# samholt/NeuralLaplaceControl

Measured on AMD Instinct MI355X. Metric: MPPI planning steps/sec (16384 samples, H=40), higher is better.
Workload: dtype f64

## Files before the change

neurallaplacecontrol_amd/csrc/abi_ctx.hip:

```cpp
#include "nlc_host.h"

using namespace nlc;
using namespace nlc::host;

namespace nlc {
namespace host {

thread_local std::string g_create_error;

bool gru_use_coop(const nlc_ctx* c, int64_t n_windows) {
  if (c->opt.gru_coop >= 0) return c->opt.gru_coop != 0;
  if (c->g == 128) return true;
  return n_windows <= (c->g == 32 ? 8192 : 50000);
}

void prof_flush(nlc_ctx* c) {
  for (auto& p : c->prof) {
    for (auto& ev : p.pending) {
      hipEventSynchronize(ev.second);
      float ms = 0.f;
      hipEventElapsedTime(&ms, ev.first, ev.second);
      p.total_ms += ms;
      c->event_pool.push_back(ev.first);
      c->event_pool.push_back(ev.second);
// ... 178 lines not shown
  } else if (n == "fused_partner_tiles") {
    if (value < -2 || value > 64) return fail(c, NLC_ERR_BAD_ARG, "fused_partner_tiles must be in -2..64 (-2 = auto, -1 = never)");
    c->opt.fused.partner_tiles = (int)value;
  } else if (n == "repfunc_split") {
    if (value != 0 && value != 1) return fail(c, NLC_ERR_BAD_ARG, "repfunc_split must be 0 or 1");
    c->opt.repfunc_split = (int)value;
  } else if (n == "gru_coop") {
    if (value != 0 && value != 1 && value != -1) return fail(c, NLC_ERR_BAD_ARG, "gru_coop must be -1 (auto), 0 or 1");
    c->opt.gru_coop = (int)value;
  } else if (n == "gru_prefix") {
    if (value != 0 && value != 1 && value != -1) return fail(c, NLC_ERR_BAD_ARG, "gru_prefix must be -1 (auto), 0 or 1");
    c->opt.gru_prefix = (int)value;
  } else if (n == "gru_gemm") {
    if (value != 0 && value != 1) return fail(c, NLC_ERR_BAD_ARG, "gru_gemm must be 0 (FP64 MFMA) or 1 (int8-sliced)");
    c->opt.gru_gemm = (int)value;
    if (c->has_model) c->gru.use_i8 = (c->gru.i8_stream != nullptr && value == 1) ? 1 : 0;
  } else if (n == "dbg_gap_us") {
    if (value < 0 || value > 1.0e5) return fail(c, NLC_ERR_BAD_ARG, "dbg_gap_us must be in 0 .. 1e5");
    c->opt.dbg_gap_us = value;
  } else if (n == "dbg_l2_mb") {
    if (value < 0 || value > 4096) return fail(c, NLC_ERR_BAD_ARG, "dbg_l2_mb must be in 0 .. 4096");
    c->opt.dbg_l2_mb = value;
  } else if (n == "fused_max_samples") {
    if (value < 0) return fail(c, NLC_ERR_BAD_ARG, "fused_max_samples must be >= 0");
    c->opt.fused_max_samples = (int64_t)value;
  } else {
    return fail(c, NLC_ERR_BAD_ARG, "unknown option: " + n);
  }
  return NLC_OK;
}

extern "C" int nlc_get_stat(nlc_ctx* c, const char* name, double* out) {
  if (!c) return NLC_ERR_BAD_ARG;
  if (!name || !out) return fail(c, NLC_ERR_BAD_ARG, "NULL stat name / out");
  const std::string n(name);
  if (n == "rollout_body") *out = (double)c->last_body;
  else if (n == "fused_timeouts") *out = (double)c->fused.timeouts;
  else if (n == "fused_fallbacks") *out = (double)c->fused.fallbacks;
  else if (n == "fused_lost") *out = c->fused.lost ? 1.0 : 0.0;
  else if (n == "last_giveup_command") *out = (double)c->fused.last_giveup_command;
  else if (n == "commands") *out = (double)c->commands;
  else if (n == "comm_world") *out = c->comm ? (double)c->comm_world : 0.0;
  else if (n == "comm_rank") *out = c->comm ? (double)c->comm_rank : -1.0;
  else if (n == "fused_blocks_per_cu") *out = (double)c->fused.blocks_per_cu;
  else if (n == "fused_spin_limit") *out = (double)c->opt.fused_spin_limit;
  else if (n == "model_nt3") *out = c->has_model ? (double)c->net.nt3 : 0.0;
  else if (n == "gru_gemm") *out = (c->has_model && c->gru.use_i8) ? 1.0 : 0.0;
  else if (n == "gru_prefix") *out = c->prefix.last_used ? 1.0 : 0.0;
  else if (n.rfind("gru_prefix_windows_l", 0) == 0 && n.size() == 21 && n[20] >= '0' && n[20] <= '4') {
    *out = 0.0;
    if (c->prefix.last_used && c->prefix.lists) {
      unsigned cnt[nlc::prefix::kLists] = {0};
      NLC_HIP(c, hipStreamSynchronize(c->stream));
      NLC_HIP(c, hipMemcpy(cnt, c->prefix.lists, sizeof(cnt), hipMemcpyDeviceToHost));
      *out = (double)cnt[n[20] - '0'];
    }
  } else if (n == "gru_prefix_table_tiles") {
    *out = 0.0;
    if (c->prefix.last_used && c->prefix.lists) {
      unsigned cnt[nlc::prefix::kLists] = {0};
      NLC_HIP(c, hipStreamSynchronize(c->stream));
      NLC_HIP(c, hipMemcpy(cnt, c->prefix.lists, sizeof(cnt), hipMemcpyDeviceToHost));
      for (int l = 1; l < nlc::prefix::n_lists(c->prefix.last_B); ++l) *out += (double)((cnt[l] + 15u) / 16u);
    }
  } else if (n == "latents_offset") *out = (c->has_mppi && c->pd.dynamics == NLC_DYN_NL) ? (double)ws_layout(c).pa : -1.0;
  else if (n == "gru_i8_launches") *out = (double)nlc::gru_i8_launch_count();
  else return fail(c, NLC_ERR_BAD_ARG, "unknown stat: " + n);
  return NLC_OK;
}

extern "C" int nlc_synchronize(nlc_ctx* c) {
  if (!c) return NLC_ERR_BAD_ARG;
  NLC_HIP(c, hipStreamSynchronize(c->stream));
  return NLC_OK;
}

extern "C" int nlc_device_info(nlc_ctx* c, char* name, int name_len, int* cus, int* mhz, double* gib) {
  if (!c) return NLC_ERR_BAD_ARG;
  if (name && name_len > 0) {
    std::snprintf(name, name_len, "%s (%s)", c->prop.name, c->prop.gcnArchName);
  }
  if (cus) *cus = c->prop.multiProcessorCount;
  if (mhz) *mhz = c->prop.clockRate / 1000;
  if (gib) *gib = (double)c->prop.totalGlobalMem / (1024.0 * 1024.0 * 1024.0);
  return NLC_OK;
}

extern "C" int nlc_profile_enable(nlc_ctx* c, int on) {
  if (!c) return NLC_ERR_BAD_ARG;
  if (!on) prof_flush(c);
  c->profiling = on != 0;
  return NLC_OK;
}
extern "C" int nlc_profile_reset(nlc_ctx* c) {
  if (!c) return NLC_ERR_BAD_ARG;
  prof_flush(c);
  c->prof.clear();
  return NLC_OK;
}
extern "C" int nlc_profile_count(nlc_ctx* c) {
  if (!c) return NLC_ERR_BAD_ARG;
  return (int)c->prof.size();
}
extern "C" int nlc_profile_read(nlc_ctx* c, int idx, char* name, int name_len, double* total_ms, int64_t* launches) {
  if (!c) return NLC_ERR_BAD_ARG;
  if (idx < 0 || idx >= (int)c->prof.size()) return fail(c, NLC_ERR_BAD_ARG, "profile index out of range");
  prof_flush(c);
  const ProfEntry& p = c->prof[idx];
  if (name && name_len > 0) std::snprintf(name, name_len, "%s", p.name.c_str());
  if (total_ms) *total_ms = p.total_ms;
  if (launches) *launches = p.launches;
  return NLC_OK;
}
```

neurallaplacecontrol_amd/csrc/abi_planner.hip:

```cpp
#include "nlc_host.h"

using namespace nlc;
using namespace nlc::host;

extern "C" int nlc_mppi_configure(nlc_ctx* c, const nlc_mppi_desc* d) {
  if (!c) return NLC_ERR_BAD_ARG;
  NLC_GUARD_BEGIN
  if (!d) return fail(c, NLC_ERR_BAD_ARG, "NULL desc");
  if (d->K < 1 || d->T < 1 || d->K_global < d->K || d->k_offset < 0 || d->k_offset + d->K > d->K_global)
    return fail(c, NLC_ERR_BAD_SHAPE, "bad K / K_global / k_offset / T");
  if (d->nu < 1 || d->nu > NLC_MAX_NU) return fail(c, NLC_ERR_UNSUPPORTED, "nu must be 1 or 2");
  if (d->d < 1 || (d->d > NLC_MAX_D && d->dynamics != NLC_DYN_EXTERNAL)) return fail(c, NLC_ERR_BAD_SHAPE, "bad nx");
  if (d->B < 1) return fail(c, NLC_ERR_BAD_SHAPE, "action_buffer needs at least one row");
  if (!(d->lambda_ > 0.0) || d->u_scale == 0.0) return fail(c, NLC_ERR_BAD_ARG, "lambda_ must be > 0, u_scale != 0");
  if (d->u_per_command < 1 || d->u_per_command > d->T) return fail(c, NLC_ERR_BAD_ARG, "bad u_per_command");
  if (d->E < 0 || d->E > 65535) return fail(c, NLC_ERR_BAD_ARG, "episodes E must be in [0, 65535]");
  const int E = d->E < 1 ? 1 : d->E;
  if ((double)E * (double)d->K * d->T * d->nu > 2.0e9)
    return fail(c, NLC_ERR_BAD_SHAPE, "E*K*T*nu exceeds the planner's index range");
  const bool env_free = d->cost_external &&
                        (d->dynamics == NLC_DYN_NL || d->dynamics == NLC_DYN_DTRNN || d->dynamics == NLC_DYN_NODE) &&
                        d->env == -1;
  if (!env_free && (d->env < 0 || d->env > NLC_ENV_CARTPOLE_NOTRIG)) return fail(c, NLC_ERR_UNSUPPORTED, "unknown env id");
  static const int env_d[4] = {5, 3, 6, 4}, env_nu[4] = {1, 1, 2, 1};
// ... 142 lines not shown
  }
  if (g.lost_here || (g.marked && count_marked)) c->fused.last_giveup_command = command;
  return g;
}

WeightArgs make_weight_args(nlc_ctx* c, const nlc_mppi_buffers* buf) {
  const nlc_mppi_desc& d = c->pd;
  const WsLayout w = ws_layout(c);
  double* ws = (double*)buf->workspace;
  WeightArgs wa{};
  wa.Kep = d.K;
  wa.E = d.E;
  wa.T = d.T;
  wa.nu = d.nu;
  wa.lambda_ = d.lambda_;
  wa.cost = buf->cost_total;
  wa.noise = buf->noise;
  wa.tile_part = ws + w.tile_part;
  wa.chunk_part = ws + w.chunk_part;
  wa.partials = buf->partials;
  wa.nblk = c->nblk;
  return wa;
}

int finish_rollout_costs(nlc_ctx* c, const nlc_mppi_buffers* buf, bool in_body) {
  const nlc_mppi_desc& d = c->pd;
  if (d.cost_external) return NLC_OK;
  if (cost_variant_of(d) && !in_body) {
    if (!buf->states) return fail(c, NLC_ERR_BAD_ARG, "this rollout body evaluates a cost_variant on buf->states");
    VariantCostArgs v{d.K * d.E, d.T, d.nu, d.d, d.env, cost_variant_of(d), d.u_scale, buf->states, buf->perturbed, buf->cost_total};
    ProfScope ps(c, "variant_cost_kernel");
    NLC_HIP(c, launch_variant_cost(v, c->stream));
  }
  return run_weights(c, buf);
}

int run_weights(nlc_ctx* c, const nlc_mppi_buffers* buf) {
  WeightArgs wa = make_weight_args(c, buf);
  if (c->last_body == 3 && buf->workspace && c->pd.dynamics == NLC_DYN_NL)
    wa.gave_up = reinterpret_cast<const unsigned*>((const double*)buf->workspace + ws_layout(c).sync) + kFusedTimeout;
  ProfScope ps(c, "weight_kernels");
  NLC_HIP(c, launch_weights(wa, c->stream));
  return NLC_OK;
}

int launch_shift_perturb(nlc_ctx* c, RolloutCall& call) {
  PerturbArgs& p = call.p;
  p.fused_shift = (int64_t)p.K * p.T > 0;
  if (!p.fused_shift) {
    ProfScope ps(c, "shift_U_kernel");
    NLC_HIP(c, launch_shift_U(p, c->stream));
  }
  ProfScope ps(c, "perturb_kernel");
  NLC_HIP(c, launch_perturb(p, c->stream));
  return NLC_OK;
}

SampleCostArgs sample_cost_args(const nlc_ctx* c, const RolloutCall& call) {
  const nlc_mppi_desc& d = c->pd;
  SampleCostArgs a{};
  a.K = call.KE;
  a.Kep = d.K;
  a.T = d.T;
  a.nu = d.nu;
  a.env = (d.cost_external || cost_variant_of(d)) ? -1 : d.env;
  a.state_per_sample = call.state_per_sample;
  a.state0 = call.state_dev;
  a.perturbed = call.buf->perturbed;
  a.noise = call.buf->noise;
  a.U = c->U[c->ucur];
  for (int i = 0; i < NLC_MAX_NU * NLC_MAX_NU; ++i) a.sigma_inv[i] = d.noise_sigma_inv[i];
  a.lambda_ = d.lambda_;
  a.u_scale = d.u_scale;
  a.noise_abs_cost = d.noise_abs_cost;
  a.states = call.buf->states;
  a.cost_total = call.buf->cost_total;
  return a;
}

PerturbArgs perturb_args(const nlc_ctx* c, const nlc_mppi_buffers* buf, int rng, uint64_t seed, uint64_t counter) {
  const nlc_mppi_desc& d = c->pd;
  PerturbArgs p{};
  p.K = d.K * d.E;
  p.Kep = d.K;
  p.E = d.E;
  p.K_global = d.K_global;
  p.k_offset = d.k_offset;
  p.T = d.T;
  p.nu = d.nu;
  p.U_old = c->U[c->ucur];
  p.U_new = c->U[c->ucur ^ 1];
  p.noise = buf->noise;
  p.perturbed = buf->perturbed;
  p.actions = buf->actions;
  p.u_scale = d.u_scale;
  p.has_bounds = d.has_bounds;
  p.sample_null_action = d.sample_null_action;
  p.rng = rng;
  for (int i = 0; i < NLC_MAX_NU; ++i) {
    p.u_min[i] = d.u_min[i];
    p.u_max[i] = d.u_max[i];
    p.u_init[i] = d.u_init[i];
    p.mu[i] = d.noise_mu[i];
  }
  for (int i = 0; i < NLC_MAX_NU * NLC_MAX_NU; ++i) p.chol[i] = d.noise_chol[i];
  p.seed = seed;
  p.counter = counter;
// ... 370 lines not shown
```

neurallaplacecontrol_amd/csrc/abi_planner_nl.hip:

```cpp
#include "nlc_host.h"

using namespace nlc;
using namespace nlc::host;

namespace {

__global__ void dbg_spin_kernel(unsigned long long ticks_100mhz) {
  const unsigned long long t0 = __builtin_amdgcn_s_memrealtime();
  while (__builtin_amdgcn_s_memrealtime() - t0 < ticks_100mhz) __builtin_amdgcn_s_sleep(8);
}
__global__ void dbg_touch_kernel(const double* __restrict__ p, size_t n, double* __restrict__ sink) {
  double acc = 0.0;
  for (size_t i = (size_t)blockIdx.x * blockDim.x + threadIdx.x; i < n; i += (size_t)gridDim.x * blockDim.x) acc += p[i];
  if (acc == 12345.678) *sink = acc;
}
int dbg_between(nlc_ctx* c) {
  if (c->opt.dbg_gap_us > 0.0) hipLaunchKernelGGL(dbg_spin_kernel, dim3(1), dim3(64), 0, c->stream, (unsigned long long)(c->opt.dbg_gap_us * 100.0));
  if (c->opt.dbg_l2_mb > 0.0) {
    const size_t bytes = (size_t)(c->opt.dbg_l2_mb * 1048576.0);
    const size_t n = bytes / 8 + 1;
    if (c->dbg_scratch_n < n) {
      if (int rc = hold_doubles(c, c->dbg_scratch, n, nullptr, &c->dbg_scratch_n)) return rc;
      NLC_HIP(c, hipMemsetAsync(c->dbg_scratch, 0, n * sizeof(double), c->stream));
    }
// ... 291 lines not shown
  f.g.N = KE * d.T;
  FusedCtl& fc = f.ctl;
  fc.sync = reinterpret_cast<unsigned*>(ws + w.sync);
  fc.timeout_host = pin_giveup_word(c);
  fc.ntk = s.ntk;
  fc.n_enc = s.n_enc;
  fc.roll_cap = s.roll_cap;
  fc.adaptive_q8 = s.adaptive_q8;
  fc.pool_wgs = s.pool_wgs;
  fc.chain_first_tiles = s.chain_first_tiles;
  fc.partner_tiles = s.partner_tiles;
  fc.spin_limit = (unsigned)c->opt.fused_spin_limit;
  fc.test_drop_tile = c->opt.fused_test_drop_tile;
  fc.inline_weights = (c->opt.fused_inline & 1) && d.E == 1 && !d.cost_external;
  fc.inline_perturb = (c->opt.fused_inline & 2) && d.E == 1 && inline_inputs && rng == 1 && d.B <= kFusedMaxInlineB;
  unsigned* sync_words = reinterpret_cast<unsigned*>(ws + w.sync);
  const size_t n_sync = fused_sync_words(d.T, KE);
  if (fc.inline_perturb) {
    if (c->fused.sync_clean_ws != buf->workspace) NLC_HIP(c, hipMemsetAsync(sync_words, 0, n_sync * sizeof(unsigned), c->stream));
  } else {
    p.zero_words = sync_words;
    p.n_zero_words = (int64_t)n_sync;
    if (int rc = launch_shift_perturb(c, call)) return rc;
  }
  c->fused.sync_clean_ws = nullptr;
  c->fused.sync_dirty = true;
  c->fused.last.fused = true;
  c->last_body = 3;
  f.p = p;
  if (fc.inline_weights) f.w = make_weight_args(c, buf);
  {
    ProfScope ps(c, "nl_plan_fused_kernel");
    NLC_HIP(c, launch_nl_plan_fused(f, c->g, s.grid, s.built, c->stream));
  }
  *weights_done = fc.inline_weights != 0;
  return NLC_OK;
}

int gru_prefix_begin(nlc_ctx* c, RolloutCall& call, const GruArgs& g, int64_t N, int chunks, bool* use, GruPrefixArgs* px) {
  *use = false;
  if (c->opt.gru_prefix == 0) return NLC_OK;
  GruPrefixState& ps = c->prefix;
  const char* why = ps.why_not;
  if (!why && ps.last_B != g.B) why = "gru_prefix: the table was built for another action-buffer length";
  if (!why && chunks != 1) why = "gru_prefix: not with the encoder in horizon chunks (horizon_chunks)";
  if (!why && gru_use_coop(c, N)) why = "gru_prefix: this launch takes the cooperative encoder (gru_coop)";
  if (!why && g.use_i8) why = "gru_prefix: the FP64 encoder only (gru_gemm is 1)";
  if (!why) why = prefix::out_of_scope(g.nact, g.nin, 1, g.B, N, true);
  if (why) return c->opt.gru_prefix == 1 ? fail(c, NLC_ERR_UNSUPPORTED, why) : NLC_OK;
  const int64_t stride = (N + 63) / 64 * 64;
  const size_t need = 64 + (size_t)prefix::kLists * (size_t)stride / 2;
  if (need > ps.lists_n) {
    NLC_HIP(c, hipStreamSynchronize(c->stream));
    if (int rc = hold_doubles(c, ps.lists, need, nullptr, &ps.lists_n)) return rc;
  }
  double* base = c->arena.base + ps.arena_off;
  px->table = base;
  px->out_tab = base + (size_t)prefix::kEntries * 2 * c->g;
  px->products = base + gru_prefix_products_off(c->g);
  px->counts = reinterpret_cast<unsigned*>(ps.lists);
  px->lists = reinterpret_cast<unsigned*>(ps.lists + 64);
  px->list_stride = stride;
  px->img_max = ps.img_max;
  px->img_min = ps.img_min;
  call.p.zero_words = px->counts;
  call.p.n_zero_words = 16;
  *use = true;
  return NLC_OK;
}

int rollout_nl_two_launch(nlc_ctx* c, RolloutCall& call, GruArgs& g, RolloutArgs& r, int variant) {
  const nlc_mppi_desc& d = c->pd;
  const int64_t KE = call.KE;
  bool use_prefix = false;
  GruPrefixArgs px{};
  {
    const int chunks = plan::horizon_chunks((variant != 2 && KE > 8192 && d.E == 1) ? c->opt.horizon_chunks : 1, d.T).C;
    if (int rc = gru_prefix_begin(c, call, g, KE * d.T, chunks, &use_prefix, &px)) return rc;
  }
  if (int rc2 = nlc::host::launch_shift_perturb(c, call)) return rc2;
  const plan::Chunks ck = plan::horizon_chunks((variant != 2 && KE > 8192 && d.E == 1) ? c->opt.horizon_chunks : 1, d.T);
  const int C = ck.C, Tc = ck.Tc;
  if (C == 1) {
    g.t0 = 0;
    g.Tc = d.T;
    g.N = KE * d.T;
    if (use_prefix) {
      {
        ProfScope ps(c, "gru_prefix_index_kernel");
        NLC_HIP(c, launch_gru_prefix_index(g, px, c->stream));
      }
      ProfScope ps(c, "gru_encode_kernel");
      NLC_HIP(c, launch_gru_encode_prefix(g, px, c->g, c->stream));
      c->prefix.last_used = true;
    } else {
      ProfScope ps(c, "gru_encode_kernel");
      NLC_HIP(c, launch_gru_encode(g, c->g, c->stream, gru_use_coop(c, g.N)));
    }
    if (c->opt.dbg_gap_us > 0.0 || c->opt.dbg_l2_mb > 0.0)
      if (int rc3 = dbg_between(c)) return rc3;
    r.t_begin = 0;
    r.t_end = d.T;
    ProfScope ps(c, "nl_rollout_kernel");
    NLC_HIP(c, launch_nl_rollout(r, c->stream, variant));
  } else {
    if (int rc = gru_encode_chunks(c, g, KE, C, Tc, false, 0u)) return rc;
    for (int ch = 0; ch < C; ++ch) {
      r.t_begin = ch * Tc;
      r.t_end = (r.t_begin + Tc <= d.T) ? r.t_begin + Tc : d.T;
      if (r.t_begin >= r.t_end) break;
      NLC_HIP(c, hipStreamWaitEvent(c->stream, c->side.ev_gru[ch], 0));
      ProfScope ps(c, "nl_rollout_kernel");
      NLC_HIP(c, launch_nl_rollout(r, c->stream, 1));
    }
  }
  return NLC_OK;
}

}

int nlc::host::gru_prefix_configure(nlc_ctx* c) {
  const nlc_mppi_desc& d = c->pd;
  GruPrefixState& ps = c->prefix;
  ps.last_B = d.B;
  ps.last_used = false;
  const double img[2] = {prefix::bound_image(d.u_max[0], d.u_scale), prefix::bound_image(d.u_min[0], d.u_scale)};
  bool finite = true;
  for (double v : img) finite = finite && std::isfinite((d.u_scale * v - c->gru.mean[0]) / c->gru.std[0]);
  ps.why_not = prefix::out_of_scope(d.nu, c->md.nin, d.has_bounds, d.B, 0, finite);
  if (ps.why_not) return NLC_OK;
  ps.img_max = prefix::bits_of(img[0]);
  ps.img_min = prefix::bits_of(img[1]);
  std::vector<double> syn((size_t)16 * d.B, 0.0);
  for (int col = 0; col < 16; ++col)
    for (int s = 0; s < prefix::cap(d.B); ++s) syn[(size_t)col * d.B + (d.B - 1 - s)] = img[(col >> s) & 1];
  double* base = c->arena.base + ps.arena_off;
  GruPrefixArgs px{};
  px.table = base;
  px.out_tab = base + (size_t)prefix::kEntries * 2 * c->g;
  px.products = base + gru_prefix_products_off(c->g);
  double* syn_dev = px.out_tab + 64;
  NLC_HIP(c, hipMemcpy(syn_dev, syn.data(), syn.size() * sizeof(double), hipMemcpyHostToDevice));
  GruArgs a = c->gru;
  a.mode = 1;
  a.perturbed = syn_dev;
  a.abuf = syn_dev;
  a.u_scale = d.u_scale;
  a.T = a.Tc = d.B;
  a.t0 = 0;
  a.Kep = 16;
  a.N = 16;
  a.B = d.B;
  a.nact = 1;
  a.out = nullptr;
  NLC_HIP(c, launch_gru_prefix_table(a, px, c->g, c->stream));
  NLC_HIP(c, hipStreamSynchronize(c->stream));
  return NLC_OK;
}

int nlc::host::rollout_nl(nlc_ctx* c, RolloutCall& call) {
  const nlc_mppi_desc& d = c->pd;
  const nlc_mppi_buffers* buf = call.buf;
  const WsLayout& w = call.w;
  double* ws = call.ws;
  const int64_t KE = call.KE;
  const bool replay = call.replay;
  const bool lin_direct = linear_on_rollout_kernels(c);
  double* pa = ws + w.pa;
  GruArgs g = c->gru;
  g.mode = 1;
  g.perturbed = buf->perturbed;
  g.abuf = call.abuf_dev;
  g.u_scale = d.u_scale;
  g.T = d.T;
  g.B = d.B;
  g.Kep = d.K;
  g.nact = d.nu;
  g.out = pa;
// ... 58 lines not shown
```

neurallaplacecontrol_amd/csrc/kernels_mppi.hip:

```cpp
#include "nlc_device.h"
#include "nlc_env_dev.h"
#include "nlc_envcost.h"
#include "nlc_kernels.h"
#include "nlc_mppi_dev.h"

namespace nlc {

__global__ void shift_U_kernel(const PerturbArgs a) {
  const int n = a.T * a.nu;
  const double* Uo = a.U_old + (int64_t)blockIdx.x * n;
  double* Un = a.U_new + (int64_t)blockIdx.x * n;
  for (int i = threadIdx.x; i < n; i += blockDim.x) {
    const int t = i / a.nu, j = i - t * a.nu;
    Un[i] = (t + 1 < a.T) ? Uo[i + a.nu] : a.u_init[j];
  }
  if (blockIdx.x == 0) {
    for (int i = threadIdx.x; i < a.n_state_in; i += blockDim.x) a.state_dst[i] = a.state_in[i];
    for (int i = threadIdx.x; i < a.n_abuf_in; i += blockDim.x) a.abuf_dst[i] = a.abuf_in[i];
  }
}
hipError_t launch_shift_U(const PerturbArgs& a, hipStream_t s) {
  hipLaunchKernelGGL(shift_U_kernel, dim3((unsigned)a.E), dim3(128), 0, s, a);
  return hipGetLastError();
}

__global__ __launch_bounds__(256) void perturb_kernel(const PerturbArgs a) {
  const int64_t total = a.K * a.T;
  for (int64_t i = (int64_t)blockIdx.x * blockDim.x + threadIdx.x; i < a.n_zero_words; i += (int64_t)gridDim.x * blockDim.x)
    a.zero_words[i] = 0u;
  if (a.fused_shift && blockIdx.x == 0) {
    for (int i = threadIdx.x; i < a.n_state_in; i += blockDim.x) a.state_dst[i] = a.state_in[i];
    for (int i = threadIdx.x; i < a.n_abuf_in; i += blockDim.x) a.abuf_dst[i] = a.abuf_in[i];
  }
  for (int64_t idx = (int64_t)blockIdx.x * blockDim.x + threadIdx.x; idx < total;
       idx += (int64_t)gridDim.x * blockDim.x) {
    const int64_t k = idx / a.T;
    const int t = (int)(idx - k * a.T);
    const int64_t e = k / a.Kep;
    const int64_t ke = a.k_offset + (k - e * a.Kep);
    const int64_t kg = e * a.K_global + ke;
    double eps[NLC_MAX_NU];
    if (a.rng) {
      mppi_draw(kg, t, a.seed, a.counter, a.nu, a.mu, a.chol, eps);
    } else {
      for (int i = 0; i < a.nu; ++i) eps[i] = a.noise[idx * a.nu + i];
    }
    const bool null_action = a.sample_null_action && (ke == a.K_global - 1);
    for (int i = 0; i < a.nu; ++i) {
      double U;
      if (a.fused_shift) {
        U = (t + 1 < a.T) ? a.U_old[(e * a.T + t + 1) * a.nu + i] : a.u_init[i];
        if (k == e * a.Kep) a.U_new[(e * a.T + t) * a.nu + i] = U;
      } else {
        U = a.U_new[(e * a.T + t) * a.nu + i];
      }
      const double V = mppi_bound(U, eps[i], null_action, a.u_scale, a.has_bounds, a.u_min[i], a.u_max[i]);
      a.perturbed[idx * a.nu + i] = V;
      a.noise[idx * a.nu + i] = V - U;
      if (a.actions != nullptr) a.actions[idx * a.nu + i] = (a.u_scale * V) / a.u_scale;
    }
  }
}
hipError_t launch_perturb(const PerturbArgs& a, hipStream_t s) {
  const int64_t total = a.K * a.T;
  if (total <= 0) return hipSuccess;
  const int64_t want = (total + 255) / 256;
  const unsigned grid = (unsigned)(want < 4096 ? want : 4096);
  hipLaunchKernelGGL(perturb_kernel, dim3(grid), dim3(256), 0, s, a);
  return hipGetLastError();
}

__global__ __launch_bounds__(256) void weight_tile_kernel(const WeightArgs a) {
  const int lane = threadIdx.x & 63;
  const int64_t b = (int64_t)blockIdx.x * 4 + (threadIdx.x >> 6);
  if (b >= a.nblk) return;
  const int64_t e = blockIdx.y;
  const int64_t ks = b * kWeightTile + (lane & 15);
  const bool valid = ks < a.Kep;
  const double cost = valid ? a.cost[e * a.Kep + ks] : 0.0;
  weight_tile<MemPlain>(a, e, b, lane, cost, valid);
}
__global__ __launch_bounds__(256) void weight_rank_kernel(const WeightArgs a) {
  __shared__ double lds[kWeightRankLds];
  weight_rank<MemPlain>(a, (int64_t)blockIdx.y, lds);
  if (a.gave_up != nullptr && threadIdx.x == 0 && __hip_atomic_load(a.gave_up, __ATOMIC_RELAXED, __HIP_MEMORY_SCOPE_AGENT) != 0u)
    a.partials[(int64_t)blockIdx.y * (2 + a.T * a.nu) + 1] = kPartialInvalidEta;
}
__global__ __launch_bounds__(256) void weight_chunk_kernel(const WeightArgs a) {
  __shared__ double lds[kWeightRankLds];
  const int64_t e = blockIdx.y;
  const int j = blockIdx.x, lane = threadIdx.x & 63, TN = a.T * a.nu;
  const double beta = weight_beta<MemPlain>(a, e, lds);
  for (int i0 = 0; i0 < 1 + TN; i0 += 64) {
    const double c = weight_chunk<MemPlain>(a, e, j, i0, beta, lds);
    if (threadIdx.x < 64 && i0 + lane < 1 + TN) a.chunk_part[(e * gridDim.x + j) * (2 + TN) + 1 + i0 + lane] = c;
  }
  if (threadIdx.x == 0) a.chunk_part[(e * gridDim.x + j) * (2 + TN)] = beta;
}
__global__ __launch_bounds__(128) void weight_final_kernel(const WeightArgs a, int nch) {
#pragma clang fp contract(off)
  const int64_t e = blockIdx.y;
  const int TN = a.T * a.nu, W = 2 + TN;
  const double* cp = a.chunk_part + e * nch * W;
  for (int i = threadIdx.x; i < 1 + TN; i += 128) {
    double tot = 0.0;
    for (int j0 = 0; j0 < nch; j0 += 16) {
      double v[16];
#pragma unroll
      for (int s = 0; s < 16; ++s) v[s] = j0 + s < nch ? cp[(int64_t)(j0 + s) * W + 1 + i] : 0.0;
#pragma unroll
      for (int s = 0; s < 16; ++s)
        if (j0 + s < nch) tot += v[s];
    }
    a.partials[e * W + 1 + i] = tot;
  }
  if (threadIdx.x == 0) {
    a.partials[e * W] = cp[0];
    if (a.gave_up != nullptr && __hip_atomic_load(a.gave_up, __ATOMIC_RELAXED, __HIP_MEMORY_SCOPE_AGENT) != 0u)
      a.partials[e * W + 1] = kPartialInvalidEta;
  }
}
// ... 301 lines not shown
```

neurallaplacecontrol_amd/csrc/nlc_gru_prefix.h:

```cpp
#pragma once
#include <cstdint>

#if defined(__HIPCC__)
#define NLC_PREFIX_HD __host__ __device__
#else
#define NLC_PREFIX_HD
#endif

namespace nlc {
namespace prefix {

constexpr int kMaxLen = 4;
constexpr int kEntries = (2 << kMaxLen) - 1;
constexpr int kLists = kMaxLen + 1;
constexpr int kMaxB = 32;
constexpr int kPatternShift = 27;
constexpr int64_t kMaxWindows = (int64_t)1 << kPatternShift;

NLC_PREFIX_HD inline uint64_t bits_of(double x) {
  uint64_t u;
  __builtin_memcpy(&u, &x, sizeof(u));
  return u;
}
NLC_PREFIX_HD inline double bound_image(double bound, double u_scale) { return bound / u_scale; }
NLC_PREFIX_HD inline int cap(int B) { return B < kMaxLen ? B : kMaxLen; }
NLC_PREFIX_HD inline int n_lists(int B) { return B < kLists ? B : kLists; }
NLC_PREFIX_HD inline int entry_index(int len, int pattern) { return (1 << len) - 1 + pattern; }

struct Class {
  int len, pattern;
};
NLC_PREFIX_HD inline Class classify(const double* row, int t, int B, uint64_t img_max, uint64_t img_min) {
  Class c{0, 0};
  const int L = cap(B);
  for (int s = 0; s < L; ++s) {
    const int i = t + B - 1 - s;
    if (i < B - 1) break;
    const uint64_t v = bits_of(row[i - (B - 1)]);
    if (v == img_max) {
    } else if (v == img_min) {
      c.pattern |= 1 << s;
    } else {
      break;
    }
    c.len = s + 1;
  }
  return c;
}

NLC_PREFIX_HD inline bool starts_tile(int len, int B) { return len >= 1 && len < n_lists(B); }
NLC_PREFIX_HD inline int build_steps(int B) { return B <= kMaxLen ? B : kMaxLen + 1; }
NLC_PREFIX_HD inline int64_t products_doubles(int g) { return (int64_t)(kEntries - 1) * 6 * g; }
NLC_PREFIX_HD inline int64_t products_entry_offset(int entry, int g) { return (int64_t)(entry - 1) * 6 * g; }
NLC_PREFIX_HD inline int products_index(int layer, int j, int set, int q, int r, int g) {
  return (((layer * (g / 16) + j) * 3 + set) * 4 + q) * 4 + r;
}

NLC_PREFIX_HD inline int64_t worst_case_tiles(int64_t N, int B) { return N / 16 + n_lists(B); }

inline const char* out_of_scope(int nu, int nin, int has_bounds, int B, int64_t N, bool images_finite) {
  if (nu != 1 || nin != 1) return "gru_prefix: one action dimension and no time channel only (nu == nin == 1)";
  if (!has_bounds) return "gru_prefix: the planner has no action bounds";
  if (B > kMaxB) return "gru_prefix: action buffers of up to 32 rows only";
  if (N > kMaxWindows) return "gru_prefix: at most 2^27 windows per launch";
  if (!images_finite) return "gru_prefix: a bound's normalised image is not finite";
  return nullptr;
}

}
}
```

neurallaplacecontrol_amd/csrc/nlc_host.h:

```cpp
#pragma once
#include <dlfcn.h>
#include <hip/hip_runtime.h>

#include <time.h>

#include <cmath>
#include <cstdio>
#include <cstdlib>
#include <cstring>
#include <stdexcept>
#include <string>
#include <vector>

#include "nlc_gru_prefix.h"
#include "nlc_kernels.h"
#include "nlc_pack.h"
#include "nlc_plan.h"

namespace nlc {
int nl_pick_nt3(int need);

namespace host {

struct ProfEntry {
// ... 41 lines not shown
  double dbg_gap_us = 0.0;
  double dbg_l2_mb = 0.0;
};

struct FusedState {
  int blocks_per_cu = -1;
  int blocks_per_cu3 = -1;
  int occ_h = 0;
  bool lost = false;
  int64_t fallbacks = 0;
  int64_t timeouts = 0;
  int64_t last_giveup_command = -1;
  const void* sync_clean_ws = nullptr;
  bool sync_dirty = false;
  struct LastCommand {
    bool valid = false, inline_inputs = false, fused = false;
    int state_per_sample = 0, rng = 0;
    uint64_t seed = 0, counter = 0;
    double state_in[NLC_MAX_D] = {0};
    double abuf_in[nlc::kMaxInlineAbuf] = {0};
  } last;
  void new_problem() {
    sync_clean_ws = nullptr;
    sync_dirty = false;
    last.valid = false;
  }
  void rearm() { lost = false; }
};

struct DehoogCalib {
  int n = 0, choice = -1, pending = -1, pending_round = 0;
  double t0 = 0.0;
  float ms[3][2] = {{1e30f, 1e30f}, {1e30f, 1e30f}, {1e30f, 1e30f}};
  hipEvent_t ev[2] = {nullptr, nullptr};
  void reset() {
    n = 0;
    choice = pending = -1;
    for (auto& v : ms) v[0] = v[1] = 1e30f;
  }
  void destroy() {
    for (hipEvent_t& e : ev) {
      if (e) hipEventDestroy(e);
      e = nullptr;
    }
  }
};

struct GruPrefixState {
  size_t arena_off = 0;
  const char* why_not = "gru_prefix: planner not configured";
  unsigned long long img_max = 0, img_min = 0;
  double* lists = nullptr;
  size_t lists_n = 0;
  bool last_used = false;
  int last_B = 0;
};

struct HostWait {
  unsigned long long seq = 0;
  double hist_us[8] = {0};
  int hist_n = 0, hist_at = 0;
  double nap_margin_us = 0.0;
  void reset() {
    hist_n = hist_at = 0;
    nap_margin_us = 0.0;
  }
};

struct SideStreams {
  hipStream_t gru_stream = nullptr;
  std::vector<hipEvent_t> ev_gru;
  std::vector<hipStream_t> aux_streams;
  hipEvent_t ev_fork = nullptr;
  std::vector<hipEvent_t> ev_join;
  hipEvent_t stage_ev = nullptr;
  void destroy() {
    if (stage_ev) hipEventDestroy(stage_ev);
    if (ev_fork) hipEventDestroy(ev_fork);
    for (hipEvent_t e : ev_join) hipEventDestroy(e);
    for (hipStream_t s : aux_streams) hipStreamDestroy(s);
    for (hipEvent_t e : ev_gru) hipEventDestroy(e);
    if (gru_stream) hipStreamDestroy(gru_stream);
    *this = SideStreams{};
  }
};

}
}

struct nlc_ctx {
  int device = 0;
  hipStream_t own_stream = nullptr;
  hipStream_t stream = nullptr;
  std::string err;
  hipDeviceProp_t prop;

  bool has_model = false;
  nlc_model_desc md{};
  int g = 0, S = 0, P = 0;
  nlc::host::DeviceArena arena;
  nlc::GruArgs gru{};
  nlc::NlNetArgs net{};
  std::vector<double> W1s_host, b1_host;
  int* slot_dev = nullptr;
  double* lin_tab = nullptr;
  int lin_algo = -1, lin_S = 0;
// ... 173 lines not shown
  a.scratch = scratch;
  return a;
}

int node_substeps(double t_end, double step, double* h, int max_n);

struct Rccl {
  typedef struct { char internal[NLC_COMM_ID_BYTES]; } UniqueId;
  int (*GetUniqueId)(UniqueId*) = nullptr;
  int (*CommInitRank)(void**, int, UniqueId, int) = nullptr;
  int (*CommDestroy)(void*) = nullptr;
  int (*AllGather)(const void*, void*, size_t, int, void*, hipStream_t) = nullptr;
  const char* (*GetErrorString)(int) = nullptr;
  std::string why;
  bool ok = false;
};
Rccl* rccl();
constexpr int kNcclFloat64 = 8;

bool linear_on_rollout_kernels(const nlc_ctx* c);
struct WsLayout {
  size_t tile_part, chunk_part, pa, state0, abuf, xcarry, ccarry, fre, fim, dx, tconst, rq, sync, total;
};
WsLayout ws_layout(const nlc_ctx* c);
inline unsigned* pin_giveup_word(nlc_ctx* c) { return reinterpret_cast<unsigned*>(c->pinned + c->pin.giveup); }
inline unsigned long long* pin_seq_word(nlc_ctx* c) { return reinterpret_cast<unsigned long long*>(c->pinned + c->pin.seq); }
inline unsigned* pin_merge_status_word(nlc_ctx* c) { return reinterpret_cast<unsigned*>(c->pinned + c->pin.merge_status); }
WeightArgs make_weight_args(nlc_ctx* c, const nlc_mppi_buffers* buf);
int run_weights(nlc_ctx* c, const nlc_mppi_buffers* buf);
inline int cost_variant_of(const nlc_mppi_desc& d) {
  if (d.cost_external || !(d.cost_variant & (NLC_COST_STATE_CONSTRAINT | NLC_COST_CHANGE_GOAL))) return 0;
  return d.cost_variant;
}
template <class A>
void cost_in_body(A& a, const nlc_mppi_desc& d) {
  if (cost_variant_of(d)) {
    a.env = d.env;
    a.cost_variant = cost_variant_of(d);
  }
}
int finish_rollout_costs(nlc_ctx* c, const nlc_mppi_buffers* buf, bool in_body = false);

struct RolloutCall {
  const nlc_mppi_buffers* buf;
  PerturbArgs p;
  WsLayout w;
  double* ws;
  double* state_dev;
  double* abuf_dev;
  int64_t KE;
  int state_per_sample, rng;
  bool inline_inputs;
  bool replay;
};
int launch_shift_perturb(nlc_ctx* c, RolloutCall& call);
SampleCostArgs sample_cost_args(const nlc_ctx* c, const RolloutCall& call);
int rollout_nl(nlc_ctx* c, RolloutCall& call);
int gru_prefix_configure(nlc_ctx* c);
inline size_t gru_prefix_products_off(int g) { return (size_t)nlc::prefix::kEntries * 2 * g + 64 + (size_t)16 * nlc::prefix::kMaxB; }
inline size_t gru_prefix_arena_doubles(int g) {
  return gru_prefix_products_off(g) + (size_t)nlc::prefix::products_doubles(g);
}

}
}
```

neurallaplacecontrol_amd/csrc/nlc_kernels.h:

```cpp
#pragma once
#include <hip/hip_runtime.h>
#include <stdint.h>

#include <climits>
#include <type_traits>

#include "../../include/nlc.h"
#include "nlc_ilt_tile.h"

namespace nlc {

struct IltArgs {
  const double* theta;
  const double* phi;
  const double* t;
  double* x;
  int64_t N;
  int d, S;
  double alpha, log_tol, scale;
  const double* fre;
  const double* fim;
  double t_div;
  int t_stride;
  int rpp, iters;
// ... 346 lines not shown
struct EnvStepArgs {
  int env, friction, B, nu, delay;
  int64_t E;
  double dt;
  double* state;
  double* abuf;
  const double* action;
  double* obs;
  double* reward;
};
hipError_t launch_env_step(const EnvStepArgs& a, hipStream_t s);

struct CollectStepArgs {
  int env, friction, B, nu, delay, time_channel, ts_grid, policy, steps_per_episode, it;
  int64_t E, episode_base;
  double dt, action_noise, obs_noise, action_low, action_high;
  uint64_t seed;
  double* state;
  double* abuf;
  const double* action;
  double* ret;
  double* s0;
  double* a0;
  double* sn;
  double* ts;
};
hipError_t launch_collect_step(const CollectStepArgs& a, hipStream_t s);

constexpr int kMaxInlineAbuf = 32;
struct PerturbArgs {
  int64_t K, Kep, K_global, k_offset;
  int T, nu, E;
  const double* U_old;
  double* U_new;
  double* noise;
  double* perturbed;
  double* actions;
  double u_scale;
  int has_bounds, sample_null_action, rng;
  double u_min[NLC_MAX_NU], u_max[NLC_MAX_NU], u_init[NLC_MAX_NU], mu[NLC_MAX_NU];
  double chol[NLC_MAX_NU * NLC_MAX_NU];
  uint64_t seed, counter;
  int n_state_in, n_abuf_in;
  double* state_dst;
  double* abuf_dst;
  double state_in[NLC_MAX_D];
  double abuf_in[kMaxInlineAbuf];
  unsigned* zero_words;
  int64_t n_zero_words;
  int fused_shift;
};
hipError_t launch_shift_U(const PerturbArgs& a, hipStream_t s);
hipError_t launch_perturb(const PerturbArgs& a, hipStream_t s);

struct WeightArgs {
  int64_t Kep;
  int T, nu, E;
  double lambda_;
  const double* cost;
  const double* noise;
  double* tile_part;
  double* chunk_part;
  double* partials;
  int nblk;
  const unsigned* gave_up;
};
constexpr double kPartialInvalidEta = -1.0;
constexpr int kWeightTile = 16;
inline int weight_tiles(int64_t Kep) { return (int)((Kep + kWeightTile - 1) / kWeightTile); }
hipError_t launch_weights(const WeightArgs& a, hipStream_t s);

struct MergeArgs {
  int64_t Kep;
  int T, nu, G, rank, u_per_command, E;
  double lambda_, u_scale;
  const double* gathered;
  double* U;
  double* cost_nz;
  double* omega;
  double* action;
  double* action_pinned;
  double* beta_eta;
  const double* cost;
  unsigned* zero_words;
  int64_t n_zero_words;
  unsigned long long* seq_pinned;
  unsigned long long seq;
  unsigned* status_pinned;
};
hipError_t launch_merge(const MergeArgs& a, hipStream_t s);

constexpr int kFusedEncTicket = 0, kFusedRollTicket = 1, kFusedTimeout = 2, kFusedCensusTicket = 3;
constexpr int kFusedStatEntered = 4, kFusedStatRollStart = 5, kFusedStatRollDone = 6, kFusedStatEncDone = 7, kFusedStatExited = 8;
constexpr int kFusedTimeEntry = 9, kFusedTimeRollBeginFirst = 10, kFusedTimeRollBeginLast = 11, kFusedTimeRollEndFirst = 12,
              kFusedTimeRollEndLast = 13, kFusedTimeEncLast = 14;
constexpr int kFusedCuOcc = 16;
constexpr int kFusedCuState = 16 + 2048;
constexpr int kFusedCostDone = 16 + 4096;
constexpr int kFusedFlags = 16 + 4096 + 16;
inline size_t fused_sync_words(int T, int64_t K) { return (size_t)kFusedFlags + (size_t)(2 * T + 1) * (size_t)((K + 15) / 16); }
constexpr int kFusedMaxInlineB = 8;
struct FusedCtl {
  unsigned* sync;
  unsigned* timeout_host;
  int ntk;
  int n_enc;
// ... 87 lines not shown
```

Before: 271.5.

## Fuse GRU prefix classification into the perturb kernel with double-buffered counters

Adds a perturb_classify kernel that produces perturbed actions and, in the same pass, classifies each window's saturated-action prefix, writes full-length outputs from the table, and appends window ids to per-length lists. The separate gru_prefix_index kernel is skipped when this path runs, which removes one launch and a reread of the perturbed buffer. The list counters are double-buffered so the perturb kernel zeros the idle block, and a memset is issued only when the state is not known to be clean. The cost is a more complex kernel with shared-memory halos and ballot-based compaction, and it is limited to nu=1 with RNG and bounds enabled.

```diff
diff --git a/neurallaplacecontrol_amd/csrc/abi_ctx.hip b/neurallaplacecontrol_amd/csrc/abi_ctx.hip
--- a/neurallaplacecontrol_amd/csrc/abi_ctx.hip
+++ b/neurallaplacecontrol_amd/csrc/abi_ctx.hip
@@ -254,7 +254,7 @@
     if (c->prefix.last_used && c->prefix.lists) {
       unsigned cnt[nlc::prefix::kLists] = {0};
       NLC_HIP(c, hipStreamSynchronize(c->stream));
-      NLC_HIP(c, hipMemcpy(cnt, c->prefix.lists, sizeof(cnt), hipMemcpyDeviceToHost));
+      NLC_HIP(c, hipMemcpy(cnt, reinterpret_cast<const unsigned*>(c->prefix.lists) + 8 * c->prefix.block, sizeof(cnt), hipMemcpyDeviceToHost));
       *out = (double)cnt[n[20] - '0'];
     }
   } else if (n == "gru_prefix_table_tiles") {
@@ -262,7 +262,7 @@
     if (c->prefix.last_used && c->prefix.lists) {
       unsigned cnt[nlc::prefix::kLists] = {0};
       NLC_HIP(c, hipStreamSynchronize(c->stream));
-      NLC_HIP(c, hipMemcpy(cnt, c->prefix.lists, sizeof(cnt), hipMemcpyDeviceToHost));
+      NLC_HIP(c, hipMemcpy(cnt, reinterpret_cast<const unsigned*>(c->prefix.lists) + 8 * c->prefix.block, sizeof(cnt), hipMemcpyDeviceToHost));
       for (int l = 1; l < nlc::prefix::n_lists(c->prefix.last_B); ++l) *out += (double)((cnt[l] + 15u) / 16u);
     }
   } else if (n == "latents_offset") *out = (c->has_mppi && c->pd.dynamics == NLC_DYN_NL) ? (double)ws_layout(c).pa : -1.0;
diff --git a/neurallaplacecontrol_amd/csrc/abi_planner.hip b/neurallaplacecontrol_amd/csrc/abi_planner.hip
--- a/neurallaplacecontrol_amd/csrc/abi_planner.hip
+++ b/neurallaplacecontrol_amd/csrc/abi_planner.hip
@@ -218,7 +218,10 @@
     NLC_HIP(c, launch_shift_U(p, c->stream));
   }
   ProfScope ps(c, "perturb_kernel");
-  NLC_HIP(c, launch_perturb(p, c->stream));
+  if (call.classify)
+    NLC_HIP(c, launch_perturb_classify(p, call.pc, c->stream));
+  else
+    NLC_HIP(c, launch_perturb(p, c->stream));
   return NLC_OK;
 }
 
diff --git a/neurallaplacecontrol_amd/csrc/abi_planner_nl.hip b/neurallaplacecontrol_amd/csrc/abi_planner_nl.hip
--- a/neurallaplacecontrol_amd/csrc/abi_planner_nl.hip
+++ b/neurallaplacecontrol_amd/csrc/abi_planner_nl.hip
@@ -367,19 +367,33 @@
   const size_t need = 64 + (size_t)prefix::kLists * (size_t)stride / 2;
   if (need > ps.lists_n) {
     NLC_HIP(c, hipStreamSynchronize(c->stream));
+    ps.next_clean = false;
     if (int rc = hold_doubles(c, ps.lists, need, nullptr, &ps.lists_n)) return rc;
   }
   double* base = c->arena.base + ps.arena_off;
   px->table = base;
   px->out_tab = base + (size_t)prefix::kEntries * 2 * c->g;
   px->products = base + gru_prefix_products_off(c->g);
-  px->counts = reinterpret_cast<unsigned*>(ps.lists);
+  unsigned* blocks = reinterpret_cast<unsigned*>(ps.lists);
+  if (!ps.next_clean) NLC_HIP(c, hipMemsetAsync(blocks, 0, 16 * sizeof(unsigned), c->stream));
+  ps.next_clean = false;
+  ps.block ^= 1;
+  px->counts = blocks + 8 * ps.block;
   px->lists = reinterpret_cast<unsigned*>(ps.lists + 64);
   px->list_stride = stride;
   px->img_max = ps.img_max;
   px->img_min = ps.img_min;
-  call.p.zero_words = px->counts;
-  call.p.n_zero_words = 16;
+  call.classify = call.p.rng != 0 && N > 0;
+  if (call.classify) {
+    call.pc.px = *px;
+    call.pc.out = g.out;
+    call.pc.B = g.B;
+    call.p.zero_words = blocks + 8 * (ps.block ^ 1);
+    call.p.n_zero_words = 8;
+  } else {
+    call.p.zero_words = blocks;
+    call.p.n_zero_words = 16;
+  }
   *use = true;
   return NLC_OK;
 }
@@ -401,13 +415,14 @@
     g.Tc = d.T;
     g.N = KE * d.T;
     if (use_prefix) {
-      {
+      if (!call.classify) {
         ProfScope ps(c, "gru_prefix_index_kernel");
         NLC_HIP(c, launch_gru_prefix_index(g, px, c->stream));
       }
       ProfScope ps(c, "gru_encode_kernel");
       NLC_HIP(c, launch_gru_encode_prefix(g, px, c->g, c->stream));
       c->prefix.last_used = true;
+      c->prefix.next_clean = true;
     } else {
       ProfScope ps(c, "gru_encode_kernel");
       NLC_HIP(c, launch_gru_encode(g, c->g, c->stream, gru_use_coop(c, g.N)));
@@ -439,6 +454,7 @@
   GruPrefixState& ps = c->prefix;
   ps.last_B = d.B;
   ps.last_used = false;
+  ps.next_clean = false;
   const double img[2] = {prefix::bound_image(d.u_max[0], d.u_scale), prefix::bound_image(d.u_min[0], d.u_scale)};
   bool finite = true;
   for (double v : img) finite = finite && std::isfinite((d.u_scale * v - c->gru.mean[0]) / c->gru.std[0]);
diff --git a/neurallaplacecontrol_amd/csrc/kernels_mppi.hip b/neurallaplacecontrol_amd/csrc/kernels_mppi.hip
--- a/neurallaplacecontrol_amd/csrc/kernels_mppi.hip
+++ b/neurallaplacecontrol_amd/csrc/kernels_mppi.hip
@@ -1,6 +1,7 @@
 #include "nlc_device.h"
 #include "nlc_env_dev.h"
 #include "nlc_envcost.h"
+#include "nlc_gru_prefix.h"
 #include "nlc_kernels.h"
 #include "nlc_mppi_dev.h"
 
@@ -24,40 +25,120 @@
   return hipGetLastError();
 }
 
-__global__ __launch_bounds__(256) void perturb_kernel(const PerturbArgs a) {
-  const int64_t total = a.K * a.T;
+template <bool Store>
+__device__ __forceinline__ double perturb_element(const PerturbArgs& a, int64_t idx) {
+  const int64_t k = idx / a.T;
+  const int t = (int)(idx - k * a.T);
+  const int64_t e = k / a.Kep;
+  const int64_t ke = a.k_offset + (k - e * a.Kep);
+  const int64_t kg = e * a.K_global + ke;
+  double eps[NLC_MAX_NU];
+  if (a.rng) {
+    mppi_draw(kg, t, a.seed, a.counter, a.nu, a.mu, a.chol, eps);
+  } else {
+    for (int i = 0; i < a.nu; ++i) eps[i] = a.noise[idx * a.nu + i];
+  }
+  const bool null_action = a.sample_null_action && (ke == a.K_global - 1);
+  double V0 = 0.0;
+  for (int i = 0; i < a.nu; ++i) {
+    double U;
+    if (a.fused_shift) {
+      U = (t + 1 < a.T) ? a.U_old[(e * a.T + t + 1) * a.nu + i] : a.u_init[i];
+      if (Store && k == e * a.Kep) a.U_new[(e * a.T + t) * a.nu + i] = U;
+    } else {
+      U = a.U_new[(e * a.T + t) * a.nu + i];
+    }
+    const double V = mppi_bound(U, eps[i], null_action, a.u_scale, a.has_bounds, a.u_min[i], a.u_max[i]);
+    if (i == 0) V0 = V;
+    if (Store) {
+      a.perturbed[idx * a.nu + i] = V;
+      a.noise[idx * a.nu + i] = V - U;
+      if (a.actions != nullptr) a.actions[idx * a.nu + i] = (a.u_scale * V) / a.u_scale;
+    }
+  }
+  return V0;
+}
+__device__ __forceinline__ void perturb_side_jobs(const PerturbArgs& a) {
   for (int64_t i = (int64_t)blockIdx.x * blockDim.x + threadIdx.x; i < a.n_zero_words; i += (int64_t)gridDim.x * blockDim.x)
     a.zero_words[i] = 0u;
   if (a.fused_shift && blockIdx.x == 0) {
     for (int i = threadIdx.x; i < a.n_state_in; i += blockDim.x) a.state_dst[i] = a.state_in[i];
     for (int i = threadIdx.x; i < a.n_abuf_in; i += blockDim.x) a.abuf_dst[i] = a.abuf_in[i];
   }
+}
+__global__ __launch_bounds__(256) void perturb_kernel(const PerturbArgs a) {
+  const int64_t total = a.K * a.T;
+  perturb_side_jobs(a);
   for (int64_t idx = (int64_t)blockIdx.x * blockDim.x + threadIdx.x; idx < total;
-       idx += (int64_t)gridDim.x * blockDim.x) {
-    const int64_t k = idx / a.T;
-    const int t = (int)(idx - k * a.T);
-    const int64_t e = k / a.Kep;
-    const int64_t ke = a.k_offset + (k - e * a.Kep);
-    const int64_t kg = e * a.K_global + ke;
-    double eps[NLC_MAX_NU];
-    if (a.rng) {
-      mppi_draw(kg, t, a.seed, a.counter, a.nu, a.mu, a.chol, eps);
-    } else {
-      for (int i = 0; i < a.nu; ++i) eps[i] = a.noise[idx * a.nu + i];
-    }
-    const bool null_action = a.sample_null_action && (ke == a.K_global - 1);
-    for (int i = 0; i < a.nu; ++i) {
-      double U;
-      if (a.fused_shift) {
-        U = (t + 1 < a.T) ? a.U_old[(e * a.T + t + 1) * a.nu + i] : a.u_init[i];
-        if (k == e * a.Kep) a.U_new[(e * a.T + t) * a.nu + i] = U;
-      } else {
-        U = a.U_new[(e * a.T + t) * a.nu + i];
+       idx += (int64_t)gridDim.x * blockDim.x)
+    perturb_element<true>(a, idx);
+}
+
+constexpr int kClassifyThreads = 512;
+constexpr int kClassifyPerThread = prefix::kRunWindows / kClassifyThreads;
+__global__ __launch_bounds__(kClassifyThreads) void perturb_classify_kernel(const PerturbArgs a, const PerturbClassifyArgs pc) {
+  __shared__ double vals[prefix::kMaxHalo + prefix::kRunWindows];
+  __shared__ unsigned cnt[8], base[8];
+  const GruPrefixArgs& px = pc.px;
+  const int64_t total = a.K * a.T;
+  const int lane = threadIdx.x & 63;
+  const int nl = prefix::n_lists(pc.B);
+  perturb_side_jobs(a);
+  if (threadIdx.x < 8) cnt[threadIdx.x] = 0u;
+  const int64_t w0 = (int64_t)blockIdx.x * prefix::kRunWindows;
+  if ((int)threadIdx.x < prefix::run_halo(w0, a.T, pc.B))
+    vals[prefix::kMaxHalo - 1 - (int)threadIdx.x] = perturb_element<false>(a, w0 - 1 - (int)threadIdx.x);
+#pragma unroll
+  for (int it = 0; it < kClassifyPerThread; ++it) {
+    const int i = it * kClassifyThreads + (int)threadIdx.x;
+    if (w0 + i < total) vals[prefix::kMaxHalo + i] = perturb_element<true>(a, w0 + i);
+  }
+  __syncthreads();
+  unsigned cls[kClassifyPerThread];
+#pragma unroll
+  for (int it = 0; it < kClassifyPerThread; ++it) {
+    const int i = it * kClassifyThreads + (int)threadIdx.x;
+    const int64_t w = w0 + i;
+    int len = 7, pattern = 0;
+    if (w < total) {
+      const int tt = (int)(w % a.T);
+      const prefix::Class c = prefix::classify_back(vals + prefix::kMaxHalo + i, tt, pc.B, px.img_max, px.img_min);
+      len = c.len;
+      pattern = c.pattern;
+      if (len == pc.B) {
+        const double* o = px.out_tab + prefix::entry_index(len, pattern) * 2;
+        pc.out[w * 2 + 0] = o[0];
+        pc.out[w * 2 + 1] = o[1];
       }
-      const double V = mppi_bound(U, eps[i], null_action, a.u_scale, a.has_bounds, a.u_min[i], a.u_max[i]);
-      a.perturbed[idx * a.nu + i] = V;
-      a.noise[idx * a.nu + i] = V - U;
-      if (a.actions != nullptr) a.actions[idx * a.nu + i] = (a.u_scale * V) / a.u_scale;
+    }
+    cls[it] = (unsigned)len | ((unsigned)pattern << 3);
+    for (int l = 0; l <= prefix::kMaxLen; ++l) {
+      const unsigned long long m = __ballot(len == l);
+      if (m != 0ull && lane == __ffsll((long long)m) - 1) atomicAdd(&cnt[l], (unsigned)__popcll(m));
+    }
+  }
+  __syncthreads();
+  if (threadIdx.x <= prefix::kMaxLen) {
+    const unsigned n = cnt[threadIdx.x];
+    base[threadIdx.x] = n ? atomicAdd(px.counts + threadIdx.x, n) : 0u;
+    cnt[threadIdx.x] = 0u;
+  }
+  __syncthreads();
+#pragma unroll
+  for (int it = 0; it < kClassifyPerThread; ++it) {
+    const int64_t w = w0 + it * kClassifyThreads + (int)threadIdx.x;
+    const int len = (int)(cls[it] & 7u);
+    for (int l = 0; l < nl; ++l) {
+      const unsigned long long m = __ballot(len == l);
+      if (m == 0ull) continue;
+      const int leader = __ffsll((long long)m) - 1;
+      unsigned b = 0u;
+      if (lane == leader) b = atomicAdd(&cnt[l], (unsigned)__popcll(m));
+      b = (unsigned)__shfl((int)b, leader);
+      if (len == l) {
+        const unsigned pos = base[l] + b + (unsigned)__popcll(m & ((1ull << lane) - 1ull));
+        if ((int64_t)pos < px.list_stride) px.lists[(int64_t)l * px.list_stride + pos] = (unsigned)w | ((cls[it] >> 3) << prefix::kPatternShift);
+      }
     }
   }
 }
@@ -67,6 +148,14 @@
   const int64_t want = (total + 255) / 256;
   const unsigned grid = (unsigned)(want < 4096 ? want : 4096);
   hipLaunchKernelGGL(perturb_kernel, dim3(grid), dim3(256), 0, s, a);
+  return hipGetLastError();
+}
+hipError_t launch_perturb_classify(const PerturbArgs& a, const PerturbClassifyArgs& pc, hipStream_t s) {
+  const int64_t total = a.K * a.T;
+  if (total <= 0) return hipSuccess;
+  if (a.nu != 1 || !a.rng || !a.has_bounds || total > prefix::kMaxWindows) return hipErrorInvalidValue;
+  const unsigned grid = (unsigned)((total + prefix::kRunWindows - 1) / prefix::kRunWindows);
+  hipLaunchKernelGGL(perturb_classify_kernel, dim3(grid), dim3(kClassifyThreads), 0, s, a, pc);
   return hipGetLastError();
 }
 
diff --git a/neurallaplacecontrol_amd/csrc/nlc_gru_prefix.h b/neurallaplacecontrol_amd/csrc/nlc_gru_prefix.h
--- a/neurallaplacecontrol_amd/csrc/nlc_gru_prefix.h
+++ b/neurallaplacecontrol_amd/csrc/nlc_gru_prefix.h
@@ -30,13 +30,13 @@
 struct Class {
   int len, pattern;
 };
-NLC_PREFIX_HD inline Class classify(const double* row, int t, int B, uint64_t img_max, uint64_t img_min) {
+NLC_PREFIX_HD inline Class classify_back(const double* newest, int t, int B, uint64_t img_max, uint64_t img_min) {
   Class c{0, 0};
   const int L = cap(B);
   for (int s = 0; s < L; ++s) {
     const int i = t + B - 1 - s;
     if (i < B - 1) break;
-    const uint64_t v = bits_of(row[i - (B - 1)]);
+    const uint64_t v = bits_of(newest[-s]);
     if (v == img_max) {
     } else if (v == img_min) {
       c.pattern |= 1 << s;
@@ -46,6 +46,16 @@
     c.len = s + 1;
   }
   return c;
+}
+NLC_PREFIX_HD inline Class classify(const double* row, int t, int B, uint64_t img_max, uint64_t img_min) {
+  return classify_back(row + t, t, B, img_max, img_min);
+}
+
+constexpr int kRunWindows = 2048;
+constexpr int kMaxHalo = kMaxLen - 1;
+NLC_PREFIX_HD inline int run_halo(int64_t w0, int T, int B) {
+  const int t0 = (int)(w0 % T);
+  return t0 < cap(B) - 1 ? t0 : cap(B) - 1;
 }
 
 NLC_PREFIX_HD inline bool starts_tile(int len, int B) { return len >= 1 && len < n_lists(B); }
diff --git a/neurallaplacecontrol_amd/csrc/nlc_host.h b/neurallaplacecontrol_amd/csrc/nlc_host.h
--- a/neurallaplacecontrol_amd/csrc/nlc_host.h
+++ b/neurallaplacecontrol_amd/csrc/nlc_host.h
@@ -117,6 +117,8 @@
   unsigned long long img_max = 0, img_min = 0;
   double* lists = nullptr;
   size_t lists_n = 0;
+  int block = 0;
+  bool next_clean = false;
   bool last_used = false;
   int last_B = 0;
 };
@@ -396,6 +398,8 @@
   int state_per_sample, rng;
   bool inline_inputs;
   bool replay;
+  bool classify;
+  PerturbClassifyArgs pc;
 };
 int launch_shift_perturb(nlc_ctx* c, RolloutCall& call);
 SampleCostArgs sample_cost_args(const nlc_ctx* c, const RolloutCall& call);
diff --git a/neurallaplacecontrol_amd/csrc/nlc_kernels.h b/neurallaplacecontrol_amd/csrc/nlc_kernels.h
--- a/neurallaplacecontrol_amd/csrc/nlc_kernels.h
+++ b/neurallaplacecontrol_amd/csrc/nlc_kernels.h
@@ -422,6 +422,12 @@
 };
 hipError_t launch_shift_U(const PerturbArgs& a, hipStream_t s);
 hipError_t launch_perturb(const PerturbArgs& a, hipStream_t s);
+struct PerturbClassifyArgs {
+  GruPrefixArgs px;
+  double* out;
+  int B;
+};
+hipError_t launch_perturb_classify(const PerturbArgs& a, const PerturbClassifyArgs& pc, hipStream_t s);
 
 struct WeightArgs {
   int64_t Kep;
```

After: 271.8 (median of 6 runs). Within noise of the previous version (+0.1%).
